# Vandermode/ELD

Hardware: AMD Instinct MI355X
Metric: raw megapixels/sec (noise-synth + U-Net step) (higher is better)
Workload: dtype f32; 1 GPU; BASELINE.json configs[1]: full ELD noise model (PGRU, SonyA7S2 params) on 4x1424x2128 packed raw + U-Net fp32 train step (fwd, L1, bwd, Adam), 8 frames per GPU; images_per_gpu=8, global_batch=8, parallelism=dp1

## Files before the change

### eld_amd/csrc/conv_x3.hip

```cpp
#include <stdlib.h>
#include "conv.h"

#include "conv_x3_dev.h"

namespace {

template <int BN, int RPW, bool DB, bool BFIRST = false, bool BSLAB = false, bool STREAM = false>
__global__ __launch_bounds__(256, 2) void conv_x3_kernel(const ConvArgs a) {
    constexpr int CK = 16;
    constexpr int TH = 4 * RPW, NT = BN / 32, A_PIX = (TH + 2) * (TW + 2);
    constexpr int A_WORDS = A_PIX * PX, B_ROWS = 3 * BN;
    extern __shared__ __attribute__((aligned(16))) float lds[];
    float* ldsA = lds;
    float* ldsB = lds + A_WORDS;

    const int tid = threadIdx.x, lane = tid & 63, wave = tid >> 6;
    const int m = lane & 31, hi = lane >> 5;
    const int NB = a.Nout / BN;
    const int Cin = a.C0 + a.C1;
    const int total_tiles = a.tiles_x * a.tiles_y * a.N * NB;
    const int Cs0 = a.C0;

    constexpr int A_UNITS = A_PIX * 4, B_UNITS = BSLAB ? B_ROWS * 7 : B_ROWS * 4;
    constexpr int A_IT = (A_UNITS + 255) / 256, B_IT = (B_UNITS + 255) / 256;
// ... 205 lines not shown
#pragma unroll
                    for (int r = 0; r < RPW; ++r) {
                        const int y = y0 + wave * RPW + r;
                        if (y >= a.H) continue;
                        const size_t pix = (size_t)(img * a.H + y) * a.W + x;
#pragma unroll
                        for (int tt = 0; tt < NT; ++tt)
                            a.codes_out[(pix * (size_t)(a.Nout >> 5) + (size_t)(nb * NT + tt)) * 2 + hi] = slope_codes16(acc[r][tt]);
                    }
                }
            }
            unsigned cw[RPW][NT];
            if (a.epi != EPI_FWD && (a.codes0 != nullptr || a.codes1 != nullptr)) {
#pragma unroll
                for (int r = 0; r < RPW; ++r) {
                    const int y = y0 + wave * RPW + r;
                    const size_t pix = (size_t)(img * a.H + (y < a.H ? y : 0)) * a.W + (xok ? x : 0);
#pragma unroll
                    for (int tt = 0; tt < NT; ++tt) {
                        const int nb32 = nb * BN + tt * 32;
                        const bool lo = nb32 < a.split;
                        const unsigned* cd = lo ? a.codes0 : a.codes1;
                        const int C = lo ? a.split : a.Nout - a.split, cb = lo ? nb32 : nb32 - a.split;
                        cw[r][tt] = cd != nullptr ? cd[(pix * (size_t)(C >> 5) + (size_t)(cb >> 5)) * 2 + hi] : 0u;
                    }
                }
            }
#pragma unroll
            for (int r = 0; r < RPW; ++r) {
                const int y = y0 + wave * RPW + r;
                const bool yok = y < a.H;
                const size_t rowpix = (size_t)(img * a.H + (yok ? y : 0)) * a.W;
                const size_t pix = rowpix + (xok ? x : 0);
#pragma unroll
                for (int tt = 0; tt < NT; ++tt) {
                    const int nb32 = nb * BN + tt * 32;
                    float4 v[4];
#pragma unroll
                    for (int q = 0; q < 4; ++q) v[q] = make_float4(acc[r][tt][4 * q], acc[r][tt][4 * q + 1], acc[r][tt][4 * q + 2], acc[r][tt][4 * q + 3]);
                    float* blk;
                    int C;
                    if (a.epi == EPI_FWD) {
                        C = a.Nout;
                        blk = static_cast<float*>(a.out0) + (rowpix + x0) * C + nb32;
                    } else {
                        const bool lo = nb32 < a.split;
                        C = lo ? a.split : a.Nout - a.split;
                        const int cb = lo ? nb32 : nb32 - a.split;
                        blk = static_cast<float*>(lo ? a.out0 : a.out1) + (rowpix + x0) * C + cb;
                        const float* act = static_cast<const float*>(lo ? a.act0 : a.act1);
                        if ((lo ? a.codes0 : a.codes1) != nullptr) {
                            const unsigned w = cw[r][tt];
#pragma unroll
                            for (int q = 0; q < 4; ++q) {
                                v[q].x *= slope_of_code(w, 4 * q); v[q].y *= slope_of_code(w, 4 * q + 1);
                                v[q].z *= slope_of_code(w, 4 * q + 2); v[q].w *= slope_of_code(w, 4 * q + 3);
                            }
                        } else if (act != nullptr) {
                            float4 s[4];
#pragma unroll
                            for (int q = 0; q < 4; ++q) s[q] = *reinterpret_cast<const float4*>(act + pix * C + cb + 4 * hi + 8 * q);
#pragma unroll
                            for (int q = 0; q < 4; ++q) {
                                v[q].x *= lrelu_slope(s[q].x); v[q].y *= lrelu_slope(s[q].y);
                                v[q].z *= lrelu_slope(s[q].z); v[q].w *= lrelu_slope(s[q].w);
                            }
                        }
                    }
                    f32_line_store(v, blk, (size_t)C, lane, yok, a.W - x0, (ELD_DBG(a) & 128) != 0);
                }
            }
        }
        if (a.epi == EPI_FWD && a.pool_out != nullptr && !(ELD_DBG(a) & 1)) {
            int img_p[RPW / 2], y_p[RPW / 2];
#pragma unroll
            for (int rp = 0; rp < RPW / 2; ++rp) { img_p[rp] = img; y_p[rp] = y0 + wave * RPW + 2 * rp; }
            pool_epilogue<RPW, NT, BN, false>(a, acc, img_p, nb, y_p, x0 + m, hi);
        }
        if (t_next >= total_tiles) break;
        t = t_next;
    }
}

template <int BN, int RPW, int WAVES, bool DB, int STREAM = 0>
__global__ __launch_bounds__(64 * WAVES, (WAVES == 4 && BN <= 64) ? 2 : (WAVES == 8 ? 2 : 1)) void conv_x3d_kernel(const ConvArgs a) {
    constexpr int CK = 16, THREADS = 64 * WAVES;
    constexpr int TH = WAVES * RPW, NT = BN / 32, A_PIX = (TH + 2) * (TW + 2);
    constexpr int B_ROWS = 3 * BN;
    constexpr bool CODES = NT <= 2;
    constexpr int B_WORDS = (B_ROWS * PX * 4 + 1023) / 1024 * 256;
    constexpr int B_PIECES = B_WORDS * 4 / 1024;
    constexpr int DMA_IT = (B_PIECES + WAVES - 1) / WAVES;
    extern __shared__ __attribute__((aligned(16))) float lds[];
    float* ldsB = lds;
    float* ldsA = lds + 2 * B_WORDS;

    const int tid = threadIdx.x, lane = tid & 63;
    const int wave = __builtin_amdgcn_readfirstlane(tid >> 6);
    const int m = lane & 31, hi = lane >> 5;
    const int NB = a.Nout / BN;
    const int Cin = a.C0 + a.C1, NCH = Cin / CK;
    constexpr bool SPLITK = WAVES == 4;
    const int KS = SPLITK && a.ksplit > 1 ? a.ksplit : 1;
    const int total_tiles = a.tiles_x * a.tiles_y * NB * KS;
    const int Cs0 = a.C0;
    const int THL = a.tile_h, TWL = a.tile_w, HWL = TWL + 2;
    const int APX = (THL + 2) * HWL, NPX = THL * TWL, VP = a.vp;
    const bool seam = VP % THL != 0;
    const bool grouped = conv_slots_grouped(THL, TWL, TH);
    const unsigned mag_hw = (unsigned)((0x100000000ull + (unsigned)HWL - 1) / (unsigned)HWL);
    const unsigned mag_tw = (unsigned)((0x100000000ull + (unsigned)TWL - 1) / (unsigned)TWL);

    constexpr int A_UNITS = A_PIX * 4;
    constexpr int A_IT = (A_UNITS + THREADS - 1) / THREADS;
    float4 ra[A_IT];
    constexpr unsigned OOB = 0xFFFFFFF0u;
    unsigned a_voff[A_IT];
    int l_img = 0;
    const unsigned ldsB_addr = (unsigned)__builtin_amdgcn_readfirstlane((int)(size_t)(__attribute__((address_space(3))) float*)ldsB);
    const unsigned long long wbase = (unsigned long long)a.wp;
    const i32x4 rsrc_w = {(int)(unsigned)wbase, (int)((unsigned)(wbase >> 32) & 0xFFFFu), (int)((size_t)3 * NCH * NB * B_WORDS * 4), 0x00020000};
    const unsigned dma_voff = (unsigned)lane * 16u;

    auto decode = [&](int t, int& nb, int& img0, int& vrel, int& x0) {
        nb = t % NB;
        const int r = t / NB;
        const int ty = r / a.tiles_x, tx = r - ty * a.tiles_x;
        const int v0 = ty * THL;
        img0 = v0 / VP; vrel = v0 - img0 * VP;
        x0 = tx * TWL;
    };
    auto strip_row = [&](int row, int& dimg, int& y) -> bool {
        const bool over = row >= VP;
        dimg = over ? 1 : 0;
        y = over ? row - VP : row;
        return over ? seam && y < a.H : (unsigned)row < (unsigned)a.H;
    };
    auto setup_load = [&](int t) {
        int nb, vrel, x0;
        decode(t, nb, l_img, vrel, x0);
#pragma unroll
        for (int it = 0; it < A_IT; ++it) {
            const int u = tid + it * THREADS;
            const int hp = stage_row(u >> 2, A_PIX), part = u & 3;
            const int hy = (int)__umulhi((unsigned)hp, mag_hw), hx = hp - hy * HWL;
            int dimg, y;
            const bool rok = strip_row(vrel + hy - 1, dimg, y);
            const int gx = x0 + hx - 1;
            const bool ok = u < A_UNITS && hp < APX && rok && gx >= 0 && gx < a.W;
            a_voff[it] = ok ? (unsigned)((dimg * a.H + y) * a.W + gx) * (unsigned)((ELD_DBG(a) & 32) ? 64 : Cs0 * 4) + (unsigned)part * 16u : OOB;
        }
    };
    auto load_A = [&](int c0) {
        if (ELD_DBG(a) & 4) return;
        const char* src = static_cast<const char*>(c0 < a.C0 ? a.in0 : a.in1);
        const int cs = c0 < a.C0 ? c0 : c0 - a.C0;
        const size_t img_bytes = (size_t)a.H * a.W * Cs0 * 4;
        const __amdgpu_buffer_rsrc_t rsrc_a = __builtin_amdgcn_make_buffer_rsrc((void*)(src + (size_t)l_img * img_bytes), 0,
                                                                                (int)(unsigned)(img_bytes * (size_t)(a.N - l_img < 2 ? a.N - l_img : 2)), 0x00020000);
        const int so = (ELD_DBG(a) & 32) ? (cs / 16) * a.H * a.W * 64 : cs * 4;
#pragma unroll
        for (int it = 0; it < A_IT; ++it)
            ra[it] = __builtin_bit_cast(float4, __builtin_amdgcn_raw_buffer_load_b128(rsrc_a, (int)a_voff[it], so, 0));
    };
    auto store_A = [&]() {
        if (ELD_DBG(a) & 16) return;
#pragma unroll
        for (int it = 0; it < A_IT; ++it) {
            const int u = tid + it * THREADS;
            if (u < A_UNITS) split_store(ldsA + stage_row(u >> 2, A_PIX) * PX + (u & 3) * 2, ra[it]);
        }
    };
    auto dma_B = [&](int buf, int nb, int chunk, int ky) {
        if (ELD_DBG(a) & 8) return;
        const unsigned soff = (unsigned)(((ky * NCH + chunk) * NB + nb) * (B_WORDS * 4));
#pragma unroll
        for (int it = 0; it < DMA_IT; ++it) {
            const int piece = wave + it * WAVES;
            if (piece < B_PIECES) bdma16(rsrc_w, dma_voff, soff + (unsigned)(piece * 1024), ldsB_addr + (unsigned)(buf * B_WORDS * 4 + piece * 1024));
        }
    };

    int pb[RPW];
#pragma unroll
    for (int r = 0; r < RPW; ++r) {
        int p = (wave * RPW + r) * 32 + conv_slot_of_lane(m, grouped);
        p = p < NPX ? p : 0;
        const int tr = (int)__umulhi((unsigned)p, mag_tw);
        pb[r] = (tr * HWL + (p - tr * TWL)) * PX + hi * 4;
    }
    auto chunk_begin = [&](int t) { return ((t % KS) * NCH) / KS; };
    auto chunk_end = [&](int t) { return ((t % KS + 1) * NCH) / KS; };
    int t = xcd_block(a.xcd);
    if (t >= total_tiles) return;
    setup_load(t / KS);
    load_A(chunk_begin(t) * CK);
    int buf = 0;
    bool after_epi = false;
    {
        int nb0, i0, v00, x00;
        decode(t / KS, nb0, i0, v00, x00);
        dma_B(0, nb0, chunk_begin(t), 0);
    }
    for (;;) {
        int nb, img0, vrel, x0;
        decode(t / KS, nb, img0, vrel, x0);
        const int t_next = t + gridDim.x;
        const int c_begin = chunk_begin(t), c_end = chunk_end(t);
        f32x16 acc[RPW][NT];
#pragma unroll
        for (int r = 0; r < RPW; ++r)
#pragma unroll
            for (int tt = 0; tt < NT; ++tt)
#pragma unroll
                for (int i = 0; i < 16; ++i) acc[r][tt][i] = 0.f;

        for (int chunk = c_begin; chunk < c_end; ++chunk) {
            const bool last_chunk = chunk + 1 >= c_end;
#pragma unroll 1
            for (int ky = 0; ky < 3; ++ky) {
                __builtin_amdgcn_s_setprio(3);
                if ((ELD_DBG(a) & 2048) && after_epi) after_epi = false;
                else
                dma_wait();
                __syncthreads();
                if (ky == 0) {
                    store_A();
                    __syncthreads();
                }
                if (ky < 2) dma_B(buf ^ 1, nb, chunk, ky + 1);
                else if (!last_chunk) dma_B(buf ^ 1, nb, chunk + 1, 0);
                else if (t_next < total_tiles) dma_B(buf ^ 1, (t_next / KS) % NB, chunk_begin(t_next), 0);
                if (ky == 0) {
                    if (!last_chunk) load_A((chunk + 1) * CK);
                    else if (t_next < total_tiles) { setup_load(t_next / KS); load_A(chunk_begin(t_next) * CK); }
                }
                __builtin_amdgcn_s_setprio(0);
                if (ELD_DBG(a) & 2) { buf ^= 1; continue; }
                const float* lb = ldsB + buf * B_WORDS;
                if constexpr (STREAM) {
                    x3_stage_blocks<RPW, NT, STREAM == 2>(acc,
                        [&](int kx, int r, uint4 (&X)[3]) {
                            const float* p = ldsA + pb[r] + (ky * HWL + kx) * PX;
#pragma unroll
                            for (int pc = 0; pc < 3; ++pc) X[pc] = *reinterpret_cast<const uint4*>(p + pc * 8);
                        },
                        [&](int kx, int tt, uint4 (&Wt)[3]) {
                            const float* p = lb + (kx * BN + tt * 32 + m) * PX + hi * 4;
#pragma unroll
                            for (int pc = 0; pc < 3; ++pc) Wt[pc] = *reinterpret_cast<const uint4*>(p + pc * 8);
                        });
                    buf ^= 1;
                    continue;
                }
                uint4 fx[DB ? 2 : 1][3][RPW], fw[DB ? 2 : 1][3][NT];
                auto read_tap = [&](int kx, uint4 (&X)[3][RPW], uint4 (&Wt)[3][NT]) {
#pragma unroll
                    for (int r = 0; r < RPW; ++r) {
                        const float* p = ldsA + pb[r] + (ky * HWL + kx) * PX;
#pragma unroll
                        for (int pc = 0; pc < 3; ++pc) X[pc][r] = *reinterpret_cast<const uint4*>(p + pc * 8);
                    }
#pragma unroll
                    for (int tt = 0; tt < NT; ++tt) {
                        const float* p = lb + (kx * BN + tt * 32 + m) * PX + hi * 4;
#pragma unroll
                        for (int pc = 0; pc < 3; ++pc) Wt[pc][tt] = *reinterpret_cast<const uint4*>(p + pc * 8);
                    }
                };
                constexpr int WI[6] = {0, 1, 2, 0, 1, 0};
                constexpr int XI[6] = {2, 1, 0, 1, 0, 0};
                if constexpr (DB) {
                    read_tap(0, fx[0], fw[0]);
#pragma unroll
                    for (int kx = 0; kx < 3; ++kx) {
                        const int cur = kx & 1;
                        if (kx + 1 < 3) read_tap(kx + 1, fx[cur ^ 1], fw[cur ^ 1]);
                        __builtin_amdgcn_sched_barrier(0);
#pragma unroll
                        for (int r = 0; r < RPW; ++r)
#pragma unroll
                            for (int j = 2; j >= 0; --j)
#pragma unroll
                                for (int i = 0; i + j <= 2; ++i)
#pragma unroll
                                    for (int tt = 0; tt < NT; ++tt)
                                        acc[r][tt] = __builtin_amdgcn_mfma_f32_32x32x16_bf16(__builtin_bit_cast(bf16x8, fw[cur][i][tt]),
                                                                                             __builtin_bit_cast(bf16x8, fx[cur][j][r]), acc[r][tt], 0, 0, 0);
                        __builtin_amdgcn_sched_barrier(0);
                    }
                } else {
#pragma unroll
                    for (int kx = 0; kx < 3; ++kx) {
                        read_tap(kx, fx[0], fw[0]);
#pragma unroll
                        for (int q = 0; q < 6; ++q)
#pragma unroll
                            for (int r = 0; r < RPW; ++r)
#pragma unroll
                                for (int tt = 0; tt < NT; ++tt)
                                    acc[r][tt] = __builtin_amdgcn_mfma_f32_32x32x16_bf16(__builtin_bit_cast(bf16x8, fw[0][WI[q]][tt]),
                                                                                         __builtin_bit_cast(bf16x8, fx[0][XI[q]][r]), acc[r][tt], 0, 0, 0);
                    }
                }
                buf ^= 1;
            }
        }

        auto slot_pixel = [&](int r, int col, size_t& pix) -> bool {
            const int p = (wave * RPW + r) * 32 + conv_slot_of_lane(col, grouped);
            const int tr = (int)__umulhi((unsigned)p, mag_tw), x = x0 + p - tr * TWL;
            int dimg, y;
            const bool ok = strip_row(vrel + tr, dimg, y) && p < NPX && img0 + dimg < a.N && x < a.W;
            pix = ok ? (size_t)((img0 + dimg) * a.H + y) * a.W + x : 0;
            return ok;
        };
        if (ELD_DBG(a) & 1) {
        } else if (KS > 1) {
            float* pbase = a.kpart + (size_t)(t % KS) * ((size_t)a.N * a.H * a.W * a.Nout);
#pragma unroll
            for (int r = 0; r < RPW; ++r) {
                size_t pix;
                if (!slot_pixel(r, m, pix)) continue;
                float* prow = pbase + pix * a.Nout + nb * BN + 4 * hi;
#pragma unroll
                for (int tt = 0; tt < NT; ++tt)
#pragma unroll
                    for (int q = 0; q < 4; ++q)
                        *reinterpret_cast<float4*>(prow + tt * 32 + 8 * q) = make_float4(acc[r][tt][4 * q], acc[r][tt][4 * q + 1], acc[r][tt][4 * q + 2], acc[r][tt][4 * q + 3]);
            }
        } else {
            if (a.epi == EPI_FWD) {
                const float sl = a.lrelu ? 0.2f : 1.0f;
#pragma unroll
                for (int tt = 0; tt < NT; ++tt)
#pragma unroll
                    for (int q = 0; q < 4; ++q) {
                        const float4 bq = *reinterpret_cast<const float4*>(a.bias + nb * BN + tt * 32 + 4 * hi + 8 * q);
#pragma unroll
                        for (int r = 0; r < RPW; ++r) bias_lrelu4(acc[r][tt], 4 * q, bq, sl);
                    }
                if (CODES && a.codes_out != nullptr) {
#pragma unroll
                    for (int r = 0; r < RPW; ++r) {
                        size_t pix;
                        if (!slot_pixel(r, m, pix)) continue;
#pragma unroll
                        for (int tt = 0; tt < NT; ++tt)
                            a.codes_out[(pix * (size_t)(a.Nout >> 5) + (size_t)(nb * NT + tt)) * 2 + hi] = slope_codes16(acc[r][tt]);
                    }
                }
            }
            const bool coded = CODES && a.epi != EPI_FWD && (a.codes0 != nullptr || a.codes1 != nullptr);
#pragma unroll
            for (int r = 0; r < RPW; ++r) {
                size_t pix, pix0, pix1;
                slot_pixel(r, m, pix);
                const bool ok0 = slot_pixel(r, lane & 15, pix0), ok1 = slot_pixel(r, (lane & 15) + 16, pix1);
                unsigned cw[NT];
                if (coded) {
#pragma unroll
                    for (int tt = 0; tt < NT; ++tt) {
                        const int nb32 = nb * BN + tt * 32;
                        const bool lo = nb32 < a.split;
                        const unsigned* cd = lo ? a.codes0 : a.codes1;
                        const int C = lo ? a.split : a.Nout - a.split, cb = lo ? nb32 : nb32 - a.split;
                        cw[tt] = cd != nullptr ? cd[(pix * (size_t)(C >> 5) + (size_t)(cb >> 5)) * 2 + hi] : 0u;
                    }
                }
#pragma unroll
                for (int tt = 0; tt < NT; ++tt) {
                    const int nb32 = nb * BN + tt * 32;
                    float4 v[4];
#pragma unroll
                    for (int q = 0; q < 4; ++q) v[q] = make_float4(acc[r][tt][4 * q], acc[r][tt][4 * q + 1], acc[r][tt][4 * q + 2], acc[r][tt][4 * q + 3]);
                    float* blk;
                    int C;
                    if (a.epi == EPI_FWD) {
                        C = a.Nout;
                        blk = static_cast<float*>(a.out0) + nb32;
                    } else {
                        const bool lo = nb32 < a.split;
                        C = lo ? a.split : a.Nout - a.split;
                        const int cb = lo ? nb32 : nb32 - a.split;
                        blk = static_cast<float*>(lo ? a.out0 : a.out1) + cb;
                        const float* act = static_cast<const float*>(lo ? a.act0 : a.act1);
                        if (CODES && (lo ? a.codes0 : a.codes1) != nullptr) {
                            const unsigned w = cw[tt];
#pragma unroll
                            for (int q = 0; q < 4; ++q) {
                                v[q].x *= slope_of_code(w, 4 * q); v[q].y *= slope_of_code(w, 4 * q + 1);
                                v[q].z *= slope_of_code(w, 4 * q + 2); v[q].w *= slope_of_code(w, 4 * q + 3);
                            }
                        } else if (act != nullptr) {
                            float4 s[4];
#pragma unroll
                            for (int q = 0; q < 4; ++q) s[q] = *reinterpret_cast<const float4*>(act + pix * C + cb + 4 * hi + 8 * q);
#pragma unroll
                            for (int q = 0; q < 4; ++q) {
                                v[q].x *= lrelu_slope(s[q].x); v[q].y *= lrelu_slope(s[q].y);
                                v[q].z *= lrelu_slope(s[q].z); v[q].w *= lrelu_slope(s[q].w);
                            }
                        }
                    }
                    f32_line_store2(v, ok0 ? blk + pix0 * C : nullptr, ok1 ? blk + pix1 * C : nullptr, lane, (ELD_DBG(a) & 128) != 0);
                }
            }
        }
        if (KS == 1 && a.epi == EPI_FWD && a.pool_out != nullptr && !(ELD_DBG(a) & 1)) {
            int img_p[RPW / 2], y_p[RPW / 2];
#pragma unroll
            for (int rp = 0; rp < RPW / 2; ++rp) {
                int dimg, y;
                const bool rok = strip_row(vrel + wave * RPW + 2 * rp, dimg, y) && img0 + dimg < a.N;
                img_p[rp] = img0 + dimg; y_p[rp] = rok ? y : a.H;
            }
            pool_epilogue<RPW, NT, BN, (WAVES == 8 && NT <= 2)>(a, acc, img_p, nb, y_p, x0 + m, hi);
        }
        if (t_next >= total_tiles) break;
        t = t_next;
        after_epi = true;
    }
}

template <int MODE, int BN, int WAVES>
__global__ __launch_bounds__(64 * WAVES, WAVES == 4 ? 2 : 1) void conv_x3_gemm_kernel(const ConvArgs a) {
    constexpr int THREADS = 64 * WAVES, RPW = 2, TH = WAVES * RPW, NT = BN / 32, NS = 2;
    constexpr int TPIX = TH * TW;
    constexpr int A_WORDS = NS * TPIX * PX;
    extern __shared__ __attribute__((aligned(16))) float lds[];
    float* ldsA = lds;
    float* ldsB = lds + A_WORDS;
    const int tid = threadIdx.x, lane = tid & 63, wave = tid >> 6;
    const int m = lane & 31, hi = lane >> 5;
    const int NB = a.Nout / BN;
    const int C0 = a.C0;
    const int Ktot = MODE == CONV_1X1 ? C0 : 4 * C0;
    const int Ws = MODE == CONV_GATHER2X2 ? 2 * a.W : a.W, Hs = MODE == CONV_GATHER2X2 ? 2 * a.H : a.H;
    const int total_tiles = a.tiles_x * a.tiles_y * a.N * NB;

    constexpr int A_UNITS = NS * TPIX * 4, B_UNITS = NS * BN * 4;
// ... 167 lines not shown
    }
}

template <bool POOL>
__global__ __launch_bounds__(256) void x3_splitk_finish_kernel(const ConvArgs a) {
    const int Q = a.Nout >> 2;
    const int Wb = POOL ? a.W >> 1 : a.W, Hb = POOL ? a.H >> 1 : a.H;
    const size_t total = (size_t)a.N * Hb * Wb * Q;
    const size_t plane = (size_t)a.N * a.H * a.W * a.Nout;
    for (size_t i = (size_t)blockIdx.x * 256 + threadIdx.x; i < total; i += (size_t)gridDim.x * 256) {
        const int q = (int)(i % Q);
        size_t p = i / Q;
        const int xb = (int)(p % Wb); p /= Wb;
        const int yb = (int)(p % Hb);
        const int img = (int)(p / Hb);
        const int n = 4 * q;
        float4 pooled = make_float4(0.f, 0.f, 0.f, 0.f);
#pragma unroll
        for (int w = 0; w < (POOL ? 4 : 1); ++w) {
            const int y = POOL ? 2 * yb + (w >> 1) : yb, x = POOL ? 2 * xb + (w & 1) : xb;
            const size_t pix = (size_t)(img * a.H + y) * a.W + x;
            float4 v = make_float4(0.f, 0.f, 0.f, 0.f);
            for (int ks = 0; ks < a.ksplit; ++ks) {
                const float4 t = *reinterpret_cast<const float4*>(a.kpart + (size_t)ks * plane + pix * a.Nout + n);
                v.x += t.x; v.y += t.y; v.z += t.z; v.w += t.w;
            }
            if (a.epi == EPI_FWD) {
                const float4 b = *reinterpret_cast<const float4*>(a.bias + n);
                v.x += b.x; v.y += b.y; v.z += b.z; v.w += b.w;
                if (a.lrelu) { v.x = fmaxf(0.2f * v.x, v.x); v.y = fmaxf(0.2f * v.y, v.y); v.z = fmaxf(0.2f * v.z, v.z); v.w = fmaxf(0.2f * v.w, v.w); }
                *reinterpret_cast<float4*>(static_cast<float*>(a.out0) + pix * a.Nout + n) = v;
                if (POOL) pooled = w == 0 ? v : make_float4(fmaxf(pooled.x, v.x), fmaxf(pooled.y, v.y), fmaxf(pooled.z, v.z), fmaxf(pooled.w, v.w));
            } else {
                const bool lo = n < a.split;
                const int C = lo ? a.split : a.Nout - a.split;
                const size_t idx = pix * C + (lo ? n : n - a.split);
                const float* act = static_cast<const float*>(lo ? a.act0 : a.act1);
                if (act) {
                    const float4 s_ = *reinterpret_cast<const float4*>(act + idx);
                    v.x *= lrelu_slope(s_.x); v.y *= lrelu_slope(s_.y); v.z *= lrelu_slope(s_.z); v.w *= lrelu_slope(s_.w);
                }
                *reinterpret_cast<float4*>(static_cast<float*>(lo ? a.out0 : a.out1) + idx) = v;
            }
        }
        if (POOL) *reinterpret_cast<float4*>(static_cast<float*>(a.pool_out) + ((size_t)(img * Hb + yb) * Wb + xb) * a.Nout + n) = pooled;
    }
}

int launch_x3_splitk_finish(const ConvArgs& a, hipStream_t st) {
    const bool pool = a.epi == EPI_FWD && a.pool_out != nullptr;
    const size_t total = (size_t)a.N * (pool ? a.H / 2 : a.H) * (pool ? a.W / 2 : a.W) * (a.Nout / 4);
    if (!total) return 0;
    const unsigned grid = (unsigned)((total + 255) / 256 < 4096 ? (total + 255) / 256 : 4096);
    if (pool) { ELD_LAUNCH(x3_splitk_finish_kernel<true>, dim3(grid), dim3(256), 0, st, a); }
    else { ELD_LAUNCH(x3_splitk_finish_kernel<false>, dim3(grid), dim3(256), 0, st, a); }
    ELD_LAUNCH_CHECK();
    return 0;
}

template <int BN, int RPW, bool DB, bool BFIRST = false, bool BSLAB = false, bool STREAM = false>
int launch_x3(ConvArgs a, hipStream_t st) {
    a.xcd = eld_xcd_mask() & XCD_X3W;
    constexpr int TH = 4 * RPW;
    a.tiles_x = (a.W + TW - 1) / TW;
    a.tiles_y = (a.H + TH - 1) / TH;
    const size_t lds_bytes = (size_t)((TH + 2) * (TW + 2) + 3 * BN) * PX * sizeof(float);
    const long long tiles = (long long)a.tiles_x * a.tiles_y * a.N * (a.Nout / BN);
    if (tiles <= 0) return 0;
    if (tiles > 0x7fffffffLL) return ELD_ENOTSUP;
    eld_note_conv_variant("conv_x3<32>", BSLAB ? nullptr : "cut", BFIRST ? nullptr : "bfirst0", STREAM ? nullptr : "stream0");
    auto kern = conv_x3_kernel<BN, RPW, DB, BFIRST, BSLAB, STREAM>;
    static EldAttrOnce once;
    { const int rc = once.ensure(kern, lds_bytes); if (rc) return rc; }
    int per_cu = (int)((160 * 1024) / lds_bytes);
    if (per_cu > 2) per_cu = 2;
    if (per_cu < 1 || (ELD_DBG(a) & 64)) per_cu = 1;
    long long grid = (long long)eld_num_cus() * per_cu;
    if (grid > tiles) grid = tiles;
    ELD_LAUNCH(kern, dim3((unsigned)grid), dim3(256), lds_bytes, st, a);
    ELD_LAUNCH_CHECK();
    return 0;
}

template <int BN, int RPW, int WAVES, bool DB, int STREAM = 0>
int launch_x3d(ConvArgs a, hipStream_t st) {
    a.xcd = eld_xcd_mask() & XCD_X3D;
    constexpr int TH = WAVES * RPW;
    conv_tile_shape(a.N, a.H, a.W, TH, a.pool_out != nullptr, a.tile_h, a.tile_w);
    a.vp = vrow_pitch(a.N, a.H, a.tile_h);
    a.tiles_x = (a.W + a.tile_w - 1) / a.tile_w;
    a.tiles_y = (vrow_extent(a.N, a.H, a.vp) + a.tile_h - 1) / a.tile_h;
    const size_t lds_bytes = (size_t)(TH + 2) * (TW + 2) * PX * sizeof(float) + 2 * (size_t)((3 * BN * PX * 4 + 1023) / 1024 * 1024);
    long long tiles = (long long)a.tiles_x * a.tiles_y * (a.Nout / BN);
    if (tiles <= 0) return 0;
    a.ksplit = 1;
    static const int no_splitk = [] { const char* e = getenv("ELD_NO_SPLITK"); return e ? atoi(e) : 0; }();
    if (WAVES == 4 && a.kpart != nullptr && !no_splitk) {
        const int nch = (a.C0 + a.C1) / 16;
        const size_t plane = (size_t)a.N * a.H * a.W * a.Nout;
        int ks = (int)(eld_num_cus() / tiles);
        if (ks > nch / 2) ks = nch / 2;
        if (ks > 16) ks = 16;
        while (ks > 1 && (size_t)ks * plane > a.kpart_floats) --ks;
        if (ks >= 2) { a.ksplit = ks; tiles *= ks; }
    }
    if (tiles > 0x7fffffffLL) return ELD_ENOTSUP;
    eld_note_conv_variant(BN == 128 ? "conv_x3d<128,8>" : (BN == 32 ? "conv_x3d<32,8>" : (WAVES == 8 ? "conv_x3d<64,8>" : (a.ksplit > 1 ? "conv_x3d<64,4,splitk>" : "conv_x3d<64,4>"))),
                          (WAVES == 8 && BN >= 64) ? (STREAM == 0 ? "stream0" : (STREAM == 1 ? "wreuse0" : nullptr)) : nullptr,
                          a.pool_out ? nullptr : conv_tile_variant());
    auto kern = conv_x3d_kernel<BN, RPW, WAVES, DB, STREAM>;
    static EldAttrOnce once;
    { const int rc = once.ensure(kern, lds_bytes); if (rc) return rc; }
    int per_cu = (int)((160 * 1024) / lds_bytes);
    if (per_cu > 2) per_cu = 2;
    if (per_cu < 1) per_cu = 1;
    long long grid = (long long)eld_num_cus() * per_cu;
    if (grid > tiles) grid = tiles;
    ELD_LAUNCH(kern, dim3((unsigned)grid), dim3(64 * WAVES), lds_bytes, st, a);
    ELD_LAUNCH_CHECK();
    if (a.ksplit > 1) return launch_x3_splitk_finish(a, st);
    return 0;
}

template <int MODE, int BN, int WAVES>
int launch_x3_gemm(ConvArgs a, hipStream_t st) {
    a.xcd = eld_xcd_mask() & XCD_GEMM;
    constexpr int TH = 2 * WAVES;
    a.tiles_x = (a.W + TW - 1) / TW;
    a.tiles_y = (a.H + TH - 1) / TH;
    const size_t lds_bytes = (size_t)(2 * TH * TW + 2 * BN) * PX * sizeof(float);
    const long long tiles = (long long)a.tiles_x * a.tiles_y * a.N * (a.Nout / BN);
    if (tiles <= 0) return 0;
    if (tiles > 0x7fffffffLL) return ELD_ENOTSUP;
    int per_cu = (int)((160 * 1024) / lds_bytes);
    if (per_cu > 2) per_cu = 2;
    long long grid = (long long)eld_num_cus() * per_cu;
    if (grid > tiles) grid = tiles;
    eld_note_conv_kernel(MODE == CONV_1X1 ? "conv_x3_gemm<1x1>" : "conv_x3_gemm<gather>");
    auto kern = conv_x3_gemm_kernel<MODE, BN, WAVES>;
    static EldAttrOnce once;
    { const int rc = once.ensure(kern, lds_bytes); if (rc) return rc; }
    ELD_LAUNCH(kern, dim3((unsigned)grid), dim3(64 * WAVES), lds_bytes, st, a);
    ELD_LAUNCH_CHECK();
    return 0;
}

}


static bool x3_32_slabs() {
    static const int on = [] { const char* e = getenv("ELD_X3_BSLAB"); return e ? atoi(e) : 0; }();
    return on != 0 || x3w_enabled();
}
static bool x3d_32_kernel(int N, int H, int W) {
    static const int on = [] { const char* e = getenv("ELD_X3D_32"); return e ? atoi(e) : 0; }();
    return on && x3_32_slabs() && conv_tile_count(N, H, W, 32, false) >= 2 * eld_num_cus();
}

int x3_slab_bn(int Nout, int N, int H, int W, int* waves) {
    if (waves) *waves = 8;
    if (Nout == 32) {
        return x3_32_slabs() ? 32 : 0;
    }
    if (Nout % 64) return 0;
    const long long px_tiles = conv_tile_count(N, H, W, 16, false);
    const int cus = eld_num_cus();
    if (Nout % 128 == 0 && px_tiles * (Nout / 128) >= cus) return 128;
    if (waves && px_tiles * (Nout / 64) < cus) *waves = 4;
    return 64;
}

int eld_xcd_mask() {
    static const int m = [] { const char* e = getenv("ELD_XCD"); return e ? atoi(e) : 127; }();
    return m;
}

int eld_tile_band() {
    static const int b = [] { const char* e = getenv("ELD_TILE_BAND"); return e ? atoi(e) : 4; }();
    return b;
}

int launch_conv_x3(const ConvArgs& a_in, hipStream_t st) {
    ConvArgs a = a_in;
    a.prof = nullptr;
    if ((size_t)a.H * a.W * a.C0 * 4 >= 0xFFFFFFF0ull) return ELD_ENOTSUP;
    if (a.pool_out && (a.epi != EPI_FWD || (a.H & 1) || (a.W & 1))) return ELD_EINVAL;
    int waves = 8;
    const int bn0 = x3_slab_bn(a.Nout, a.N, a.H, a.W, nullptr);
    if ((bn0 >= 64 || (bn0 == 32 && x3d_32_kernel(a.N, a.H, a.W))) && a.N > 1 && (size_t)a.H * a.W * a.C0 * 8 >= 0xFFFFFFF0ull) return ELD_ENOTSUP;
    const int bn = x3_slab_bn(a.Nout, a.N, a.H, a.W, &waves);
    static const int stream = [] { const char* e = getenv("ELD_X3_STREAM"); return e ? atoi(e) : 7; }();
    if (bn == 32 && x3w_takes(a)) return launch_conv_x3w(a, st);
    if (bn == 32 && x3d_32_kernel(a.N, a.H, a.W)) return launch_x3d<32, 4, 8, false>(a, st);
    if (bn == 32) return (stream & 1) ? launch_x3<32, 4, false, true, true, true>(a, st) : launch_x3<32, 4, false, true, true>(a, st);
    static const int wreuse = [] { const char* e = getenv("ELD_X3_WREUSE"); return e ? atoi(e) : 6; }();
    if (bn == 128) {
        if ((stream & 4) && (wreuse & 4)) return launch_x3d<128, 2, 8, false, 2>(a, st);
        return (stream & 4) ? launch_x3d<128, 2, 8, false, 1>(a, st) : launch_x3d<128, 2, 8, false>(a, st);
    }
    if (bn == 64) {
        if (waves != 8) return launch_x3d<64, 2, 4, false>(a, st);
        if ((stream & 2) && (wreuse & 2)) return launch_x3d<64, 2, 8, false, 2>(a, st);
        return (stream & 2) ? launch_x3d<64, 2, 8, false, 1>(a, st) : launch_x3d<64, 2, 8, false>(a, st);
    }
    static const int bfirst = [] { const char* e = getenv("ELD_X3_BFIRST"); return e ? atoi(e) : 1; }();
    if (bfirst) return (stream & 1) ? launch_x3<32, 4, false, true, false, true>(a, st) : launch_x3<32, 4, false, true>(a, st);
    return launch_x3<32, 4, false>(a, st);
}

int launch_conv_x3_gemm(const ConvArgs& a, int mode, hipStream_t st) {
    const size_t src_img = (size_t)a.H * a.W * a.C0 * 4 * (mode == CONV_GATHER2X2 ? 4 : 1);
    if (a.Nout % 64 || a.C0 % 32 || a.C1 != 0 || src_img >= 0xFFFFFFF0ull) return ELD_ENOTSUP;
    if (mode == CONV_1X1 && a.epi == EPI_CONVT_FWD && a.Cout_t % 32) return ELD_ENOTSUP;
    if (mode == CONV_1X1 && a.epi == EPI_CONVT_FWD) return launch_x3_gemm<CONV_1X1, 64, 4>(a, st);
    if (mode == CONV_GATHER2X2 && a.epi == EPI_GRAD && a.split == a.Nout) return launch_x3_gemm<CONV_GATHER2X2, 64, 4>(a, st);
    return ELD_ENOTSUP;
}
```

### eld_amd/csrc/conv_x3_dev.h

```cpp
#pragma once
#include "conv.h"

namespace {

#define PX 28
#define TW 32
typedef __bf16 bf16x8 __attribute__((ext_vector_type(8)));


__device__ __forceinline__ unsigned hi_pair(unsigned lo_src, unsigned hi_src) {
    return __builtin_amdgcn_perm(hi_src, lo_src, 0x07060302u);
}

__device__ __forceinline__ void split_store(float* row, float4 v) {
    const unsigned x0 = __float_as_uint(v.x), x1 = __float_as_uint(v.y), x2 = __float_as_uint(v.z), x3 = __float_as_uint(v.w);
    const float r0 = v.x - __uint_as_float(x0 & 0xFFFF0000u), r1 = v.y - __uint_as_float(x1 & 0xFFFF0000u);
    const float r2 = v.z - __uint_as_float(x2 & 0xFFFF0000u), r3 = v.w - __uint_as_float(x3 & 0xFFFF0000u);
    const unsigned y0 = __float_as_uint(r0), y1 = __float_as_uint(r1), y2 = __float_as_uint(r2), y3 = __float_as_uint(r3);
    const float s0 = r0 - __uint_as_float(y0 & 0xFFFF0000u), s1 = r1 - __uint_as_float(y1 & 0xFFFF0000u);
    const float s2 = r2 - __uint_as_float(y2 & 0xFFFF0000u), s3 = r3 - __uint_as_float(y3 & 0xFFFF0000u);
    *reinterpret_cast<uint2*>(row) = make_uint2(hi_pair(x0, x1), hi_pair(x2, x3));
    *reinterpret_cast<uint2*>(row + 8) = make_uint2(hi_pair(y0, y1), hi_pair(y2, y3));
    *reinterpret_cast<uint2*>(row + 16) = make_uint2(hi_pair(__float_as_uint(s0), __float_as_uint(s1)), hi_pair(__float_as_uint(s2), __float_as_uint(s3)));
}


__device__ __forceinline__ int stage_row(int r, int limit) {
    const int b = r & ~7, j = r & 7;
    return b + 8 > limit ? r : b + ((j & 3) << 1) + (j >> 2);
}

template <int RPW, int NT, int BN, bool PCODES = (NT <= 2)>
__device__ __forceinline__ void pool_epilogue(const ConvArgs& a, const f32x16 (&acc)[RPW][NT], const int (&img_p)[RPW / 2], int nb,
                                              const int (&y_p)[RPW / 2] , int x, int hi) {
    static_assert(RPW % 2 == 0, "row pairs per lane");
    const int Hp = a.H >> 1, Wp = a.W >> 1;
#pragma unroll
    for (int tt = 0; tt < NT; ++tt) {
        const int nbase = nb * BN + tt * 32 + 4 * hi;
#pragma unroll
        for (int rp = 0; rp < RPW / 2; ++rp) {
            const int y = y_p[rp], img = img_p[rp];
            if (y >= a.H) continue;
            float4 pv[4];
#pragma unroll
            for (int q = 0; q < 4; ++q) {
                float u[4];
#pragma unroll
                for (int j = 0; j < 4; ++j) u[j] = fmax_lane_xor1(fmax_raw(acc[2 * rp][tt][4 * q + j], acc[2 * rp + 1][tt][4 * q + j]));
                pv[q] = make_float4(u[0], u[1], u[2], u[3]);
            }
            if (x < a.W && !(x & 1)) {
                float* dst = static_cast<float*>(a.pool_out) + ((size_t)(img * Hp + (y >> 1)) * Wp + (x >> 1)) * a.Nout + nbase;
#pragma unroll
                for (int q = 0; q < 4; ++q) *reinterpret_cast<float4*>(dst + 8 * q) = pv[q];
            }
            if constexpr (PCODES) if (a.pool_codes_out != nullptr) {
                unsigned Et = 0, Eb = 0;
#pragma unroll
                for (int i = 15; i >= 0; --i) {
                    const float mx = i % 4 == 0 ? pv[i / 4].x : (i % 4 == 1 ? pv[i / 4].y : (i % 4 == 2 ? pv[i / 4].z : pv[i / 4].w));
                    asm("v_cmp_eq_f32 vcc, %1, %2\n\tv_addc_co_u32 %0, vcc, %0, %0, vcc" : "+v"(Et) : "v"(acc[2 * rp][tt][i]), "v"(mx) : "vcc");
                    asm("v_cmp_eq_f32 vcc, %1, %2\n\tv_addc_co_u32 %0, vcc, %0, %0, vcc" : "+v"(Eb) : "v"(acc[2 * rp + 1][tt][i]), "v"(mx) : "vcc");
                }
                const unsigned Etr = (unsigned)__builtin_amdgcn_update_dpp(0, (int)Et, 0xB1, 0xF, 0xF, true);
                const unsigned Vb = ~(Et | Etr), Hb = ~Et & (Etr | ~Eb);
                if (x < a.W && !(x & 1))
                    a.pool_codes_out[((((size_t)(img * Hp + (y >> 1)) * Wp + (x >> 1)) * (size_t)(a.Nout >> 5)) + (size_t)((nb * BN + tt * 32) >> 5)) * 2 + hi] = (Vb & 0xFFFFu) | (Hb << 16);
            }
        }
    }
}

typedef int i32x4 __attribute__((ext_vector_type(4)));
__device__ __forceinline__ void bdma16(i32x4 rsrc, unsigned voff, unsigned soff, unsigned lds_dst) {
    unsigned keep;
    asm volatile("s_nop 4\n\ts_mov_b32 %0, m0\n\ts_mov_b32 m0, %4\n\ts_nop 0\n\tbuffer_load_dwordx4 %1, %2, %3 offen lds\n\ts_mov_b32 m0, %0"
                 : "=&s"(keep) : "v"(voff), "s"(rsrc), "s"(soff), "s"(lds_dst) : "memory");
}
__device__ __forceinline__ void dma_wait() { asm volatile("s_waitcnt vmcnt(0)" ::: "memory"); }

template <int RPW, int NT, bool WREUSE = false, typename RX, typename RW>
__device__ __forceinline__ void x3_stage_blocks(f32x16 (&acc)[RPW][NT], RX&& readX, RW&& readW) {
    constexpr int NBLK = 3 * RPW * NT;
    constexpr int WI[6] = {0, 1, 2, 0, 1, 0};
    constexpr int XI[6] = {2, 1, 0, 1, 0, 0};
    if constexpr (WREUSE && NT > 1) {
        uint4 X[RPW][3], Wf[2][3];
        readX(0, 0, X[0]);
        readW(0, 0, Wf[0]);
#pragma unroll
        for (int b = 0; b < NBLK; ++b) {
            const int tt = (b / RPW) % NT, r = b % RPW;
            const int wi = (b / RPW) & 1;
            if (b + 1 < NBLK) {
                const int kx1 = (b + 1) / (RPW * NT), tt1 = ((b + 1) / RPW) % NT, r1 = (b + 1) % RPW;
                if (tt1 == 0) readX(kx1, r1, X[r1]);
                if (r1 == 0) readW(kx1, tt1, Wf[wi ^ 1]);
            }
            __builtin_amdgcn_sched_barrier(0);
#pragma unroll
            for (int q = 0; q < 6; ++q)
                acc[r][tt] = __builtin_amdgcn_mfma_f32_32x32x16_bf16(__builtin_bit_cast(bf16x8, Wf[wi][WI[q]]), __builtin_bit_cast(bf16x8, X[r][XI[q]]), acc[r][tt], 0, 0, 0);
            __builtin_amdgcn_sched_barrier(0);
        }
        return;
    }
    uint4 X[2][3], Wf[2][3];
    readX(0, 0, X[0]);
    readW(0, 0, Wf[0]);
#pragma unroll
    for (int b = 0; b < NBLK; ++b) {
        const int kx = b / (RPW * NT), r = (b / NT) % RPW, tt = b % NT;
        const int xi = (b / NT) & 1;
        const int wi = NT > 1 ? (b & 1) : ((b / RPW) & 1);
        if (b + 1 < NBLK) {
            const int kx1 = (b + 1) / (RPW * NT), r1 = ((b + 1) / NT) % RPW, tt1 = (b + 1) % NT;
            if (kx1 != kx || r1 != r) readX(kx1, r1, X[xi ^ 1]);
            if (kx1 != kx || tt1 != tt) readW(kx1, tt1, Wf[wi ^ 1]);
        }
        __builtin_amdgcn_sched_barrier(0);
#pragma unroll
        for (int q = 0; q < 6; ++q)
            acc[r][tt] = __builtin_amdgcn_mfma_f32_32x32x16_bf16(__builtin_bit_cast(bf16x8, Wf[wi][WI[q]]), __builtin_bit_cast(bf16x8, X[xi][XI[q]]), acc[r][tt], 0, 0, 0);
        __builtin_amdgcn_sched_barrier(0);
    }
}

}
```

Before: 716.9 raw MPix/s.

## Overlap bf16x3 split of next A tile with MFMA blocks in conv_x3d

After: 710.3 raw MPix/s. Within noise of the previous version (-0.9%).

```diff
diff --git a/eld_amd/csrc/conv_x3.hip b/eld_amd/csrc/conv_x3.hip
--- a/eld_amd/csrc/conv_x3.hip
+++ b/eld_amd/csrc/conv_x3.hip
@@ -311,7 +311,7 @@
     }
 }
 
-template <int BN, int RPW, int WAVES, bool DB, int STREAM = 0>
+template <int BN, int RPW, int WAVES, bool DB, int STREAM = 0, bool AHEAD = false>
 __global__ __launch_bounds__(64 * WAVES, (WAVES == 4 && BN <= 64) ? 2 : (WAVES == 8 ? 2 : 1)) void conv_x3d_kernel(const ConvArgs a) {
     constexpr int CK = 16, THREADS = 64 * WAVES;
     constexpr int TH = WAVES * RPW, NT = BN / 32, A_PIX = (TH + 2) * (TW + 2);
@@ -343,6 +343,8 @@
     constexpr int A_UNITS = A_PIX * 4;
     constexpr int A_IT = (A_UNITS + THREADS - 1) / THREADS;
     float4 ra[A_IT];
+    constexpr int NA = AHEAD ? A_IT : 0;
+    unsigned rp[NA ? NA : 1][6];
     constexpr unsigned OOB = 0xFFFFFFF0u;
     unsigned a_voff[A_IT];
     int l_img = 0;
@@ -365,12 +367,17 @@
         y = over ? row - VP : row;
         return over ? seam && y < a.H : (unsigned)row < (unsigned)a.H;
     };
+    auto fresh = [&](int v) {
+        if constexpr (AHEAD) asm volatile("" : "+v"(v));
+        return v;
+    };
     auto setup_load = [&](int t) {
         int nb, vrel, x0;
         decode(t, nb, l_img, vrel, x0);
+        const int tid_s = fresh(tid);
 #pragma unroll
         for (int it = 0; it < A_IT; ++it) {
-            const int u = tid + it * THREADS;
+            const int u = tid_s + it * THREADS;
             const int hp = stage_row(u >> 2, A_PIX), part = u & 3;
             const int hy = (int)__umulhi((unsigned)hp, mag_hw), hx = hp - hy * HWL;
             int dimg, y;
@@ -389,8 +396,10 @@
                                                                                 (int)(unsigned)(img_bytes * (size_t)(a.N - l_img < 2 ? a.N - l_img : 2)), 0x00020000);
         const int so = (ELD_DBG(a) & 32) ? (cs / 16) * a.H * a.W * 64 : cs * 4;
 #pragma unroll
-        for (int it = 0; it < A_IT; ++it)
+        for (int it = 0; it < A_IT; ++it) {
             ra[it] = __builtin_bit_cast(float4, __builtin_amdgcn_raw_buffer_load_b128(rsrc_a, (int)a_voff[it], so, 0));
+            if constexpr (AHEAD) if (it < NA) { rp[it][0] = __float_as_uint(ra[it].x); rp[it][1] = __float_as_uint(ra[it].y); rp[it][2] = __float_as_uint(ra[it].z); rp[it][3] = __float_as_uint(ra[it].w); }
+        }
     };
     auto store_A = [&]() {
         if (ELD_DBG(a) & 16) return;
@@ -398,6 +407,27 @@
         for (int it = 0; it < A_IT; ++it) {
             const int u = tid + it * THREADS;
             if (u < A_UNITS) split_store(ldsA + stage_row(u >> 2, A_PIX) * PX + (u & 3) * 2, ra[it]);
+        }
+    };
+    auto cut_A1 = [&](int it) {
+        if (ELD_DBG(a) & 16) return;
+        uint2 p[3];
+        cut4(make_float4(__uint_as_float(rp[it][0]), __uint_as_float(rp[it][1]), __uint_as_float(rp[it][2]), __uint_as_float(rp[it][3])), p);
+        reg_pin(p);
+#pragma unroll
+        for (int k = 0; k < 3; ++k) { rp[it][2 * k] = p[k].x; rp[it][2 * k + 1] = p[k].y; }
+    };
+    auto write_A = [&]() {
+        if (ELD_DBG(a) & 16) return;
+#pragma unroll
+        for (int it = 0; it < A_IT; ++it) {
+            const int u = tid + it * THREADS;
+            float* row = ldsA + stage_row(u >> 2, A_PIX) * PX + (u & 3) * 2;
+            if (u >= A_UNITS) continue;
+            if (it < NA) {
+                const uint2 p[3] = {make_uint2(rp[it][0], rp[it][1]), make_uint2(rp[it][2], rp[it][3]), make_uint2(rp[it][4], rp[it][5])};
+                piece_store(row, p);
+            } else split_store(row, ra[it]);
         }
     };
     auto dma_B = [&](int buf, int nb, int chunk, int ky) {
@@ -431,6 +461,10 @@
         decode(t / KS, nb0, i0, v00, x00);
         dma_B(0, nb0, chunk_begin(t), 0);
     }
+    if constexpr (AHEAD) {
+#pragma unroll
+        for (int it = 0; it < NA; ++it) cut_A1(it);
+    }
     for (;;) {
         int nb, img0, vrel, x0;
         decode(t / KS, nb, img0, vrel, x0);
@@ -446,7 +480,7 @@
 
         for (int chunk = c_begin; chunk < c_end; ++chunk) {
             const bool last_chunk = chunk + 1 >= c_end;
-#pragma unroll 1
+#pragma unroll AHEAD ? 3 : 1
             for (int ky = 0; ky < 3; ++ky) {
                 __builtin_amdgcn_s_setprio(3);
                 if ((ELD_DBG(a) & 2048) && after_epi) after_epi = false;
@@ -454,8 +488,12 @@
                 dma_wait();
                 __syncthreads();
                 if (ky == 0) {
-                    store_A();
+                    if constexpr (AHEAD) write_A(); else store_A();
                     __syncthreads();
+                }
+                if constexpr (AHEAD) if (ky == 2) {
+#pragma unroll
+                    for (int it = 0; it < NA; ++it) asm volatile("" : "+v"(rp[it][0]), "+v"(rp[it][1]), "+v"(rp[it][2]), "+v"(rp[it][3]));
                 }
                 if (ky < 2) dma_B(buf ^ 1, nb, chunk, ky + 1);
                 else if (!last_chunk) dma_B(buf ^ 1, nb, chunk + 1, 0);
@@ -468,17 +506,19 @@
                 if (ELD_DBG(a) & 2) { buf ^= 1; continue; }
                 const float* lb = ldsB + buf * B_WORDS;
                 if constexpr (STREAM) {
-                    x3_stage_blocks<RPW, NT, STREAM == 2>(acc,
-                        [&](int kx, int r, uint4 (&X)[3]) {
-                            const float* p = ldsA + pb[r] + (ky * HWL + kx) * PX;
-#pragma unroll
-                            for (int pc = 0; pc < 3; ++pc) X[pc] = *reinterpret_cast<const uint4*>(p + pc * 8);
-                        },
-                        [&](int kx, int tt, uint4 (&Wt)[3]) {
-                            const float* p = lb + (kx * BN + tt * 32 + m) * PX + hi * 4;
-#pragma unroll
-                            for (int pc = 0; pc < 3; ++pc) Wt[pc] = *reinterpret_cast<const uint4*>(p + pc * 8);
-                        });
+                    auto readX = [&](int kx, int r, uint4 (&X)[3]) {
+                        const float* p = ldsA + pb[r] + (ky * HWL + kx) * PX;
+#pragma unroll
+                        for (int pc = 0; pc < 3; ++pc) X[pc] = *reinterpret_cast<const uint4*>(p + pc * 8);
+                    };
+                    auto readW = [&](int kx, int tt, uint4 (&Wt)[3]) {
+                        const float* p = lb + (kx * BN + tt * 32 + m) * PX + hi * 4;
+#pragma unroll
+                        for (int pc = 0; pc < 3; ++pc) Wt[pc] = *reinterpret_cast<const uint4*>(p + pc * 8);
+                    };
+                    static_assert(A_IT <= 3 * RPW * NT, "one staging unit per fragment block");
+                    if (AHEAD && ky == 2) x3_stage_blocks<RPW, NT, STREAM == 2, NA>(acc, readX, readW, [&](int b) { cut_A1(b); });
+                    else x3_stage_blocks<RPW, NT, STREAM == 2>(acc, readX, readW);
                     buf ^= 1;
                     continue;
                 }
@@ -522,6 +562,11 @@
 #pragma unroll
                     for (int kx = 0; kx < 3; ++kx) {
                         read_tap(kx, fx[0], fw[0]);
+                        if constexpr (AHEAD) if (ky == 2) {
+                            constexpr int PER = (NA + 2) / 3;
+#pragma unroll
+                            for (int it = kx * PER; it < (kx + 1) * PER && it < NA; ++it) cut_A1(it);
+                        }
 #pragma unroll
                         for (int q = 0; q < 6; ++q)
 #pragma unroll
@@ -536,6 +581,7 @@
             }
         }
 
+        const int lane_e = fresh(lane);
         auto slot_pixel = [&](int r, int col, size_t& pix) -> bool {
             const int p = (wave * RPW + r) * 32 + conv_slot_of_lane(col, grouped);
             const int tr = (int)__umulhi((unsigned)p, mag_tw), x = x0 + p - tr * TWL;
@@ -550,7 +596,7 @@
 #pragma unroll
             for (int r = 0; r < RPW; ++r) {
                 size_t pix;
-                if (!slot_pixel(r, m, pix)) continue;
+                if (!slot_pixel(r, lane_e & 31, pix)) continue;
                 float* prow = pbase + pix * a.Nout + nb * BN + 4 * hi;
 #pragma unroll
                 for (int tt = 0; tt < NT; ++tt)
@@ -573,7 +619,7 @@
 #pragma unroll
                     for (int r = 0; r < RPW; ++r) {
                         size_t pix;
-                        if (!slot_pixel(r, m, pix)) continue;
+                        if (!slot_pixel(r, lane_e & 31, pix)) continue;
 #pragma unroll
                         for (int tt = 0; tt < NT; ++tt)
                             a.codes_out[(pix * (size_t)(a.Nout >> 5) + (size_t)(nb * NT + tt)) * 2 + hi] = slope_codes16(acc[r][tt]);
@@ -584,8 +630,8 @@
 #pragma unroll
             for (int r = 0; r < RPW; ++r) {
                 size_t pix, pix0, pix1;
-                slot_pixel(r, m, pix);
-                const bool ok0 = slot_pixel(r, lane & 15, pix0), ok1 = slot_pixel(r, (lane & 15) + 16, pix1);
+                slot_pixel(r, lane_e & 31, pix);
+                const bool ok0 = slot_pixel(r, lane_e & 15, pix0), ok1 = slot_pixel(r, (lane_e & 15) + 16, pix1);
                 unsigned cw[NT];
                 if (coded) {
 #pragma unroll
@@ -919,7 +965,7 @@
     return 0;
 }
 
-template <int BN, int RPW, int WAVES, bool DB, int STREAM = 0>
+template <int BN, int RPW, int WAVES, bool DB, int STREAM = 0, bool AHEAD = false>
 int launch_x3d(ConvArgs a, hipStream_t st) {
     a.xcd = eld_xcd_mask() & XCD_X3D;
     constexpr int TH = WAVES * RPW;
@@ -944,8 +990,9 @@
     if (tiles > 0x7fffffffLL) return ELD_ENOTSUP;
     eld_note_conv_variant(BN == 128 ? "conv_x3d<128,8>" : (BN == 32 ? "conv_x3d<32,8>" : (WAVES == 8 ? "conv_x3d<64,8>" : (a.ksplit > 1 ? "conv_x3d<64,4,splitk>" : "conv_x3d<64,4>"))),
                           (WAVES == 8 && BN >= 64) ? (STREAM == 0 ? "stream0" : (STREAM == 1 ? "wreuse0" : nullptr)) : nullptr,
-                          a.pool_out ? nullptr : conv_tile_variant());
-    auto kern = conv_x3d_kernel<BN, RPW, WAVES, DB, STREAM>;
+                          a.pool_out ? nullptr : conv_tile_variant(),
+                          (!AHEAD && BN >= 64 && (WAVES == 4 || STREAM == 2)) ? "cut0" : nullptr);
+    auto kern = conv_x3d_kernel<BN, RPW, WAVES, DB, STREAM, AHEAD>;
     static EldAttrOnce once;
     { const int rc = once.ensure(kern, lds_bytes); if (rc) return rc; }
     int per_cu = (int)((160 * 1024) / lds_bytes);
@@ -1026,18 +1073,19 @@
     const int bn0 = x3_slab_bn(a.Nout, a.N, a.H, a.W, nullptr);
     if ((bn0 >= 64 || (bn0 == 32 && x3d_32_kernel(a.N, a.H, a.W))) && a.N > 1 && (size_t)a.H * a.W * a.C0 * 8 >= 0xFFFFFFF0ull) return ELD_ENOTSUP;
     const int bn = x3_slab_bn(a.Nout, a.N, a.H, a.W, &waves);
-    static const int stream = [] { const char* e = getenv("ELD_X3_STREAM"); return e ? atoi(e) : 7; }();
+    static const int stream = [] { const char* e = getenv("ELD_X3_STREAM"); return e ? atoi(e) : 15; }();
+    const bool ahead = (stream & 8) != 0;
     if (bn == 32 && x3w_takes(a)) return launch_conv_x3w(a, st);
     if (bn == 32 && x3d_32_kernel(a.N, a.H, a.W)) return launch_x3d<32, 4, 8, false>(a, st);
     if (bn == 32) return (stream & 1) ? launch_x3<32, 4, false, true, true, true>(a, st) : launch_x3<32, 4, false, true, true>(a, st);
     static const int wreuse = [] { const char* e = getenv("ELD_X3_WREUSE"); return e ? atoi(e) : 6; }();
     if (bn == 128) {
-        if ((stream & 4) && (wreuse & 4)) return launch_x3d<128, 2, 8, false, 2>(a, st);
+        if ((stream & 4) && (wreuse & 4)) return ahead ? launch_x3d<128, 2, 8, false, 2, true>(a, st) : launch_x3d<128, 2, 8, false, 2>(a, st);
         return (stream & 4) ? launch_x3d<128, 2, 8, false, 1>(a, st) : launch_x3d<128, 2, 8, false>(a, st);
     }
     if (bn == 64) {
-        if (waves != 8) return launch_x3d<64, 2, 4, false>(a, st);
-        if ((stream & 2) && (wreuse & 2)) return launch_x3d<64, 2, 8, false, 2>(a, st);
+        if (waves != 8) return ahead ? launch_x3d<64, 2, 4, false, 0, true>(a, st) : launch_x3d<64, 2, 4, false>(a, st);
+        if ((stream & 2) && (wreuse & 2)) return ahead ? launch_x3d<64, 2, 8, false, 2, true>(a, st) : launch_x3d<64, 2, 8, false, 2>(a, st);
         return (stream & 2) ? launch_x3d<64, 2, 8, false, 1>(a, st) : launch_x3d<64, 2, 8, false>(a, st);
     }
     static const int bfirst = [] { const char* e = getenv("ELD_X3_BFIRST"); return e ? atoi(e) : 1; }();
diff --git a/eld_amd/csrc/conv_x3_dev.h b/eld_amd/csrc/conv_x3_dev.h
--- a/eld_amd/csrc/conv_x3_dev.h
+++ b/eld_amd/csrc/conv_x3_dev.h
@@ -12,17 +12,29 @@
     return __builtin_amdgcn_perm(hi_src, lo_src, 0x07060302u);
 }
 
-__device__ __forceinline__ void split_store(float* row, float4 v) {
+__device__ __forceinline__ void cut4(float4 v, uint2 (&p)[3]) {
     const unsigned x0 = __float_as_uint(v.x), x1 = __float_as_uint(v.y), x2 = __float_as_uint(v.z), x3 = __float_as_uint(v.w);
     const float r0 = v.x - __uint_as_float(x0 & 0xFFFF0000u), r1 = v.y - __uint_as_float(x1 & 0xFFFF0000u);
     const float r2 = v.z - __uint_as_float(x2 & 0xFFFF0000u), r3 = v.w - __uint_as_float(x3 & 0xFFFF0000u);
     const unsigned y0 = __float_as_uint(r0), y1 = __float_as_uint(r1), y2 = __float_as_uint(r2), y3 = __float_as_uint(r3);
     const float s0 = r0 - __uint_as_float(y0 & 0xFFFF0000u), s1 = r1 - __uint_as_float(y1 & 0xFFFF0000u);
     const float s2 = r2 - __uint_as_float(y2 & 0xFFFF0000u), s3 = r3 - __uint_as_float(y3 & 0xFFFF0000u);
-    *reinterpret_cast<uint2*>(row) = make_uint2(hi_pair(x0, x1), hi_pair(x2, x3));
-    *reinterpret_cast<uint2*>(row + 8) = make_uint2(hi_pair(y0, y1), hi_pair(y2, y3));
-    *reinterpret_cast<uint2*>(row + 16) = make_uint2(hi_pair(__float_as_uint(s0), __float_as_uint(s1)), hi_pair(__float_as_uint(s2), __float_as_uint(s3)));
+    p[0] = make_uint2(hi_pair(x0, x1), hi_pair(x2, x3));
+    p[1] = make_uint2(hi_pair(y0, y1), hi_pair(y2, y3));
+    p[2] = make_uint2(hi_pair(__float_as_uint(s0), __float_as_uint(s1)), hi_pair(__float_as_uint(s2), __float_as_uint(s3)));
 }
+__device__ __forceinline__ void piece_store(float* row, const uint2 (&p)[3]) {
+    *reinterpret_cast<uint2*>(row) = p[0];
+    *reinterpret_cast<uint2*>(row + 8) = p[1];
+    *reinterpret_cast<uint2*>(row + 16) = p[2];
+}
+__device__ __forceinline__ void split_store(float* row, float4 v) {
+    uint2 p[3];
+    cut4(v, p);
+    piece_store(row, p);
+}
+__device__ __forceinline__ void reg_pin(float4& v) { asm volatile("" : "+v"(v.x), "+v"(v.y), "+v"(v.z), "+v"(v.w)); }
+__device__ __forceinline__ void reg_pin(uint2 (&p)[3]) { asm volatile("" : "+v"(p[0].x), "+v"(p[0].y), "+v"(p[1].x), "+v"(p[1].y), "+v"(p[2].x), "+v"(p[2].y)); }
 
 
 __device__ __forceinline__ int stage_row(int r, int limit) {
@@ -80,8 +92,16 @@
 }
 __device__ __forceinline__ void dma_wait() { asm volatile("s_waitcnt vmcnt(0)" ::: "memory"); }
 
-template <int RPW, int NT, bool WREUSE = false, typename RX, typename RW>
-__device__ __forceinline__ void x3_stage_blocks(f32x16 (&acc)[RPW][NT], RX&& readX, RW&& readW) {
+#define X3_HOOK_VALU 4
+#define X3_HOOK_SPREAD(b)                                                                                                       \
+    if ((b) < HOOK_BLOCKS) {                                                                                                    \
+        _Pragma("unroll") for (int q_ = 0; q_ < 6; ++q_) {                                                                      \
+            __builtin_amdgcn_sched_group_barrier(0x008, 1, 0);                                                                  \
+            __builtin_amdgcn_sched_group_barrier(0x002, X3_HOOK_VALU, 0);                                                       \
+        }                                                                                                                       \
+    }
+template <int RPW, int NT, bool WREUSE, int HOOK_BLOCKS, typename RX, typename RW, typename HK>
+__device__ __forceinline__ void x3_stage_blocks(f32x16 (&acc)[RPW][NT], RX&& readX, RW&& readW, HK&& hook) {
     constexpr int NBLK = 3 * RPW * NT;
     constexpr int WI[6] = {0, 1, 2, 0, 1, 0};
     constexpr int XI[6] = {2, 1, 0, 1, 0, 0};
@@ -99,9 +119,11 @@
                 if (r1 == 0) readW(kx1, tt1, Wf[wi ^ 1]);
             }
             __builtin_amdgcn_sched_barrier(0);
+            if (b < HOOK_BLOCKS) hook(b);
 #pragma unroll
             for (int q = 0; q < 6; ++q)
                 acc[r][tt] = __builtin_amdgcn_mfma_f32_32x32x16_bf16(__builtin_bit_cast(bf16x8, Wf[wi][WI[q]]), __builtin_bit_cast(bf16x8, X[r][XI[q]]), acc[r][tt], 0, 0, 0);
+            X3_HOOK_SPREAD(b)
             __builtin_amdgcn_sched_barrier(0);
         }
         return;
@@ -120,11 +142,17 @@
             if (kx1 != kx || tt1 != tt) readW(kx1, tt1, Wf[wi ^ 1]);
         }
         __builtin_amdgcn_sched_barrier(0);
+        if (b < HOOK_BLOCKS) hook(b);
 #pragma unroll
         for (int q = 0; q < 6; ++q)
             acc[r][tt] = __builtin_amdgcn_mfma_f32_32x32x16_bf16(__builtin_bit_cast(bf16x8, Wf[wi][WI[q]]), __builtin_bit_cast(bf16x8, X[xi][XI[q]]), acc[r][tt], 0, 0, 0);
+        X3_HOOK_SPREAD(b)
         __builtin_amdgcn_sched_barrier(0);
     }
 }
+template <int RPW, int NT, bool WREUSE = false, typename RX, typename RW>
+__device__ __forceinline__ void x3_stage_blocks(f32x16 (&acc)[RPW][NT], RX&& readX, RW&& readW) {
+    x3_stage_blocks<RPW, NT, WREUSE, 0>(acc, readX, readW, [](int) {});
+}
 
 }
```
